# sarath-srinivas/PyGPR

Measured on AMD Instinct MI355X. Metric: NLML+grad evals/sec at N=16384 D=8 RBF, higher is better.
Workload: dtype f64; 1 GPU; BASELINE config 3: one exact-GP NLML+gradient evaluation per GPU per step, N=16384 D=8, Compose([Squared_exponential, White_noise]), hp sigma=1 l=1 sigma_n=0.1, jitter 1e-7; N>1: grBCM shared-hp co-training (each rank's expert = 1024 global + 15360 own points), one all-reduce of [1+nhp] per step; experts_per_gpu=1

## Files before the change

### pygpr_amd/_ops.py

```python
import atexit
import ctypes as C
import os

import torch

from . import _lib
from ._lib import PAD, PG_F32, PG_F64, CovSpec

JITTER = 1e-7


def pad_to(n, q=PAD):
    return ((int(n) + q - 1) // q) * q


def _code(dtype):
    if dtype == torch.float64:
        return PG_F64
    if dtype == torch.float32:
        return PG_F32
    raise TypeError("pygpr_amd computes in float64 or float32, got %s" % dtype)


def _p(t):
# ... 354 lines not shown
            "pg_trmm_lower_kt_batched")

    def syrk_nt_sub_batched(self, vt_all, c_all, lower_only=True):
        self._chk(vt_all, c_all)
        assert vt_all.dim() == 3 and c_all.dim() == 3 and vt_all.shape[0] == c_all.shape[0]
        _lib.check(self.lib.pg_syrk_nt_sub_batched(self.h, _code(c_all.dtype), c_all.shape[1], vt_all.shape[2], _p(vt_all),
                                                   vt_all.stride(1), vt_all.stride(0), _p(c_all), c_all.stride(1), c_all.stride(0),
                                                   c_all.shape[0], int(lower_only), self._st()), "pg_syrk_nt_sub_batched")

    def grbcm_local_terms(self, mean_c, var_c, var_g, is_first, accumulate, out, beta=None, prec=None):
        self._chk(mean_c, var_c, var_g, out, beta, prec)
        assert out.dtype == torch.float64 and out.shape[0] == 3
        _lib.check(self.lib.pg_grbcm_local_terms(self.h, _code(mean_c.dtype), mean_c.numel(), _p(mean_c), _p(var_c),
                                                 _p(var_g), int(is_first), int(accumulate), _p(out), out.stride(0),
                                                 _p(beta), _p(prec), self._st()), "pg_grbcm_local_terms")

    def grbcm_local_terms_batched(self, mean_all, var_all, var_g, first, accumulate, out, beta=None, prec=None):
        self._chk(var_g, out)
        assert out.dtype == torch.float64 and out.shape[0] == 3 and mean_all.stride(-1) == 1 and var_all.stride(-1) == 1
        m = var_g.numel()
        nexp = mean_all.shape[0]
        if beta is not None:
            assert beta.stride(-1) == 1 and prec.stride(-1) == 1 and (nexp == 1 or beta.stride(0) == prec.stride(0))
        _lib.check(self.lib.pg_grbcm_local_terms_batched(
            self.h, _code(mean_all.dtype), m, _p(mean_all), mean_all.stride(0), _p(var_all), var_all.stride(0), _p(var_g), nexp, int(first),
            int(accumulate), _p(out), out.stride(0), _p(beta), _p(prec), beta.stride(0) if beta is not None else 0, self._st()),
            "pg_grbcm_local_terms_batched")

    def grbcm_finish(self, sums, mean_g, var_g, mean, var, beta0=None, prec0=None):
        self._chk(sums, mean_g, var_g, mean, var, beta0, prec0)
        _lib.check(self.lib.pg_grbcm_finish(self.h, _code(mean_g.dtype), mean_g.numel(), _p(sums), sums.stride(0),
                                            _p(mean_g), _p(var_g), _p(mean), _p(var), _p(beta0), _p(prec0),
                                            self._st()), "pg_grbcm_finish")

    def grbcm_weighted_prec(self, prec, beta, acc, m, accumulate):
        self._chk(prec, beta, acc)
        _lib.check(self.lib.pg_grbcm_weighted_prec(self.h, _code(acc.dtype), m, acc.shape[0], _p(prec), prec.stride(0), _p(beta),
                                                   _p(acc), acc.stride(0), int(accumulate), self._st()), "pg_grbcm_weighted_prec")

    def symmetrize(self, a, n):
        self._chk(a)
        _lib.check(self.lib.pg_symmetrize(self.h, _code(a.dtype), n, _p(a), a.stride(0), self._st()), "pg_symmetrize")

    def grbcm_finish_full(self, sums, mean_g, var_g, cov, mean):
        self._chk(sums, mean_g, var_g, cov, mean)
        _lib.check(self.lib.pg_grbcm_finish_full(self.h, _code(mean_g.dtype), mean_g.numel(), _p(sums), sums.stride(0), _p(mean_g),
                                                 _p(var_g), _p(cov), cov.stride(0), _p(mean), self._st()), "pg_grbcm_finish_full")

    def spd_inverse_lower(self, a_pad):
        n = a_pad.shape[0]
        invd = self.potrf_workspace(n, a_pad.dtype)
        info = torch.zeros(1, dtype=torch.int32, device=self.device)
        self.potrf(a_pad, invd, info)
        minv = self.empty(n, n, dtype=a_pad.dtype)
        self.trtri(a_pad, invd, minv)
        out = self.empty(n, n, dtype=a_pad.dtype)
        self.lauum(minv, out)
        return out, info

    def spd_inverse_lower_batched(self, a_all):
        nexp, n = a_all.shape[0], a_all.shape[1]
        invd = self.empty(nexp, self.potrf_worksize(n, a_all.dtype), dtype=a_all.dtype)
        info = torch.zeros(nexp, dtype=torch.int32, device=self.device)
        minv = self.empty(nexp, n, n, dtype=a_all.dtype)
        self.potrf_trtri_batched(a_all, invd, info, minv)
        self.lauum_batched(minv, a_all)
        return a_all, info

    def sqdist_argmin(self, x, centres, dist=None, idx=None):
        self._chk(x, centres, dist, idx)
        _lib.check(self.lib.pg_sqdist_argmin(self.h, _code(x.dtype), _p(x), x.stride(0), x.shape[0], _p(centres),
                                             centres.stride(0), centres.shape[0], x.shape[1], _p(dist),
                                             dist.stride(0) if dist is not None else 0, _p(idx), self._st()), "pg_sqdist_argmin")

    def gemm_raw(self, variant, m, n, k, alpha, a, b, beta, c, tri=0, klo=0, khi=0):
        self._chk(a, b, c)
        _lib.check(self.lib.pg_gemm_raw(self.h, _code(c.dtype), variant, m, n, k, float(alpha), _p(a), a.stride(0),
                                        _p(b), b.stride(0), float(beta), _p(c), c.stride(0), tri, klo, khi,
                                        self._st()), "pg_gemm_raw")

    def set_lookahead(self, on):
        _lib.check(self.lib.pg_set_lookahead(self.h, int(on)), "pg_set_lookahead")

    def set_outer_panel(self, columns):
        _lib.check(self.lib.pg_set_outer_panel(self.h, int(columns)), "pg_set_outer_panel")

    def set_recursive_split(self, min_n):
        _lib.check(self.lib.pg_set_recursive_split(self.h, int(min_n)), "pg_set_recursive_split")

    def set_coupled_chain(self, on):
        _lib.check(self.lib.pg_set_coupled_chain(self.h, int(on)), "pg_set_coupled_chain")

    def set_spin_budget(self, microseconds):
        _lib.check(self.lib.pg_set_spin_budget(self.h, int(microseconds)), "pg_set_spin_budget")

    def chain_timeouts(self):
        return int(self.lib.pg_chain_timeouts(self.h))

    def set_rearm_after(self, calls):
        _lib.check(self.lib.pg_set_rearm_after(self.h, int(calls)), "pg_set_rearm_after")

    def chain_rearms(self):
        return int(self.lib.pg_chain_rearms(self.h))

    def wait_budget_us(self, n):
        return int(self.lib.pg_wait_budget_us(self.h, int(n)))

    def spin_probe(self, n):
        scratch = torch.zeros(4, dtype=torch.int64, device=self.device)
        _lib.check(self.lib.pg_spin_probe(self.h, int(n), _p(scratch), self._st()), "pg_spin_probe")
        torch.cuda.synchronize()
        v = scratch.tolist()
        return v[2] * 1e-5, bool(v[3])

    def recover_from_timeout(self):
        torch.cuda.synchronize()
        self.chain_timeouts()
        if self.coupled_chain():
            _lib.check(self.lib.pg_set_coupled_chain(self.h, -1), "pg_set_coupled_chain")
        self.fallbacks = getattr(self, "fallbacks", 0) + 1

    def build_factor_checked(self, spec, hp, x, a, invd, info, minv=None, jitter=JITTER):
        passes = _passes(spec)
        assert len(passes) == 1
        self._chk(hp, x, a, invd, info, minv)
        n, d = x.shape
        out = C.c_int(0)
        _lib.check(self.lib.pg_build_potrf_trtri_checked(
            self.h, _code(a.dtype), C.byref(passes[0]), _p(hp), _p(x), x.stride(0), n, d, float(jitter), _p(a), a.stride(0),
            a.shape[0], _p(invd), _p(info), _p(minv), minv.stride(0) if minv is not None else 0, self._st(), C.byref(out)),
            "pg_build_potrf_trtri_checked")
        return out.value

    def coupled_chain(self):
        return int(self.lib.pg_coupled_chain(self.h))

    def last_coupled_panels(self):
        return int(self.lib.pg_last_coupled_panels(self.h))

    def leaf_raw(self, a, inv, info):
        self._chk(a, inv, info)
        _lib.check(self.lib.pg_leaf_raw(self.h, _code(a.dtype), _p(a), a.stride(0), _p(inv), inv.stride(0) if inv is not None else 0,
                                        _p(info), self._st()), "pg_leaf_raw")

    def profile(self, on):
        _lib.check(self.lib.pg_profile(self.h, int(on)), "pg_profile")

    def profile_read(self):
        f, ms, n = C.c_double(), C.c_double(), C.c_long()
        _lib.check(self.lib.pg_profile_read(self.h, C.byref(f), C.byref(ms), C.byref(n)), "pg_profile_read")
        return f.value, ms.value, n.value


_OPS = None


def get_ops():
    global _OPS
    if _OPS is None:
        _OPS = HipOps()
    return _OPS


def _passes(spec):
    return spec if isinstance(spec, (list, tuple)) else [spec]

# ... 20 lines not shown
```

### pygpr_amd/csrc/capi.hip

```cpp
#include "gemm.h"
#include "kbuild.h"
#include "leaf.h"
#include "chainstep.h"
#include "linalg.h"
#include <cstdarg>
#include <cstdint>
#include <cstdio>
#include <cstdlib>
#include <cstring>
#include <mutex>
#include <vector>

static thread_local char g_err[512] = "";

static std::mutex g_live_mu;
static std::vector<pg_ctx*> g_live;
static bool g_atexit_registered = false;

static void release_ctx(pg_ctx* h) {
    (void)hipStreamDestroy(h->aux);
    if (h->rows) (void)hipStreamDestroy(h->rows);
    if (h->upd) (void)hipStreamDestroy(h->upd);
    for (int i = 0; i < 8; ++i) (void)hipEventDestroy(h->ev[i]);
    for (int i = 0; i < h->npool; ++i) (void)hipEventDestroy(h->pool[i]);
// ... 123 lines not shown
static int probe_concurrent_queues(pg_ctx* c) {
    if (!c->probe_words && hipHostMalloc(reinterpret_cast<void**>(&c->probe_words), 64, hipHostMallocMapped) != hipSuccess) {
        (void)hipGetLastError();
        c->probe_words = nullptr;
        return 0;
    }
    int* words = c->probe_words;
    words[0] = 0;
    words[1] = 0;
    int* dwords = nullptr;
    int ok = 0;
    if (hipHostGetDevicePointer(reinterpret_cast<void**>(&dwords), words, 0) == hipSuccess) {
        hipLaunchKernelGGL(pg_probe_wait_kernel, dim3(1), dim3(1), 0, c->aux, dwords, dwords + 1);
        hipLaunchKernelGGL(pg_probe_set_kernel, dim3(1), dim3(1), 0, c->rows, dwords);
        if (hipStreamSynchronize(c->aux) == hipSuccess && hipStreamSynchronize(c->rows) == hipSuccess) ok = words[1] == 1;
    }
    (void)hipGetLastError();
    return ok;
}

static void maybe_rearm(pg_ctx* h) {
    if (h && h->coupled && h->rearms > 0 && h->rearm_cur > h->rearm_after && ++h->calls_since_rearm > h->rearm_cur) {
        h->rearm_cur = h->rearm_after;
        h->calls_since_rearm = 0;
    }
    if (!h || !h->tmo_off || h->coupled || h->rearm_after <= 0) return;
    if (h->rearm_cur < h->rearm_after) h->rearm_cur = h->rearm_after;
    if (++h->calls_since_tmo <= h->rearm_cur) return;
    h->calls_since_tmo = 0;
    if (h->rows && h->spin_ticks >= 0 && probe_concurrent_queues(h)) {
        h->coupled = 1;
        h->tmo_off = 0;
        h->rearms += 1;
        h->calls_since_rearm = 0;
    }
}

template <typename T>
static int build_potrf_t(pg_handle h, hipStream_t st, const pg_covspec* spec, const double* hp, const void* X, long ldx, int n, int d,
                         double jitter, void* A, long lda, int n_pad, void* inv_diag, int* info, void* Minv, long ldm) {
    BuildReq<T> br;
    br.spec = spec; br.hp = hp; br.X = (const T*)X; br.ldx = ldx; br.n_real = n; br.d = d; br.jitter = jitter;
    return pg_potrf_t<T>(h, st, n_pad, (T*)A, lda, (T*)inv_diag, info, (T*)Minv, ldm, &br);
}

template <typename T>
static int potrf_batched_t(pg_handle h, hipStream_t st, const pg_covspec* spec, const double* hp, long hp_stride, const void* X, long ldx,
                           long x_stride, int n, int d, double jitter, void* A, long lda, long a_stride, int n_pad, void* inv_diag,
                           long inv_stride, int* info, void* Minv, long ldm, long m_stride, int nexp) {
    ExpBatch eb;
    eb.nexp = nexp; eb.eA = a_stride; eb.eInv = inv_stride; eb.eM = m_stride; eb.eX = x_stride; eb.ehp = hp_stride;
    BuildReq<T> br;
    br.spec = spec; br.hp = hp; br.X = (const T*)X; br.ldx = ldx; br.n_real = n; br.d = d; br.jitter = jitter;
    return pg_potrf_t<T>(h, st, n_pad, (T*)A, lda, (T*)inv_diag, info, (T*)Minv, ldm, X ? &br : nullptr, &eb);
}

extern "C" {

int pg_version(void) { return 100; }
const char* pg_last_error(void) { return g_err; }

int pg_create(pg_handle* h) {
    NEED(h, "null handle pointer");
    int count = 0;
    if (hipGetDeviceCount(&count) != hipSuccess || count == 0) {
        pg_set_error("pg_create: no HIP device visible");
        return -101;
    }
    pg_ctx* c = new pg_ctx();
    memset(c, 0, sizeof(*c));
    int prio_lo = 0, prio_hi = 0;
    PG_CHECK(hipDeviceGetStreamPriorityRange(&prio_lo, &prio_hi));
    PG_CHECK(hipStreamCreateWithPriority(&c->aux, hipStreamNonBlocking, prio_hi));
    c->rows = nullptr;
    c->last_coupled = 0;
    c->lookahead = 1;
    {
        const char* e = getenv("PG_NBO");
        c->nbo = e ? atoi(e) : 0;
        if (c->nbo < 128 || c->nbo % 128 || c->nbo > 2048) c->nbo = 0;
        const char* r = getenv("PG_REC_MIN");
        c->rec_min = r ? atoi(r) : 16384;
        if (c->rec_min < 0 || (c->rec_min > 0 && (c->rec_min < 512 || c->rec_min % 512))) c->rec_min = 16384;
    }
    {
        hipDeviceProp_t prop;
        int dev = 0;
        PG_CHECK(hipGetDevice(&dev));
        PG_CHECK(hipGetDeviceProperties(&prop, dev));
        const int ncu = prop.multiProcessorCount;
        const int words = (ncu + 31) / 32;
        uint32_t mask[64];
        for (int i = 0; i < 64; ++i) mask[i] = 0;
        const char* env = getenv("PG_RESERVED_CUS");
        int reserved = env ? atoi(env) : PG_RESERVED_CUS;
        if (reserved < 1 || reserved > ncu / 2) reserved = PG_RESERVED_CUS;
        c->ncu = ncu; c->upd_cus = ncu - reserved;
        for (int cu = 0; cu < ncu - reserved; ++cu) mask[cu / 32] |= (1u << (cu % 32));
        if (ncu <= reserved * 2 || words > 64 ||
            hipExtStreamCreateWithCUMask(&c->upd, (uint32_t)words, mask) != hipSuccess) {
            c->upd = nullptr;
            c->lookahead = 0;
            (void)hipGetLastError();
        }
    }
    {
        const char* envr = getenv("PG_ROWS_STREAM");
        c->rows = nullptr;
        if (!(envr && !atoi(envr)) && c->upd &&
            hipStreamCreateWithPriority(&c->rows, hipStreamNonBlocking, prio_hi) != hipSuccess) {
            c->rows = nullptr;
            (void)hipGetLastError();
        }
    }
    c->coupled = (c->rows && probe_concurrent_queues(c)) ? 1 : 0;
    {
        c->tmo_host = nullptr;
        c->tmo_dev = nullptr;
        if (hipHostMalloc(reinterpret_cast<void**>(&c->tmo_host), 64, hipHostMallocMapped) == hipSuccess) {
            c->tmo_host[0] = 0;
            if (hipHostGetDevicePointer(reinterpret_cast<void**>(&c->tmo_dev), c->tmo_host, 0) != hipSuccess) c->tmo_dev = nullptr;
        }
        (void)hipGetLastError();
        const char* e = getenv("PG_CS_SPIN_US");
        const long long us = e ? atoll(e) : 0;
        c->spin_ticks = us < 0 ? -1 : us * 100;
        c->timeouts = 0;
        const char* ra = getenv("PG_CS_REARM");
        c->rearm_after = ra ? std::max(0, atoi(ra)) : 8;
        c->rearm_cur = c->rearm_after;
    }
    for (int i = 0; i < 8; ++i) PG_CHECK(hipEventCreate(&c->ev[i]));
    {
        std::lock_guard<std::mutex> lk(g_live_mu);
        g_live.push_back(c);
        if (!g_atexit_registered) {
            atexit(destroy_live_handles);
            g_atexit_registered = true;
        }
    }
    *h = c;
    return 0;
}

int pg_destroy(pg_handle h) {
    if (!h) return 0;
    {
        std::lock_guard<std::mutex> lk(g_live_mu);
        auto it = std::find(g_live.begin(), g_live.end(), h);
        if (it == g_live.end()) return 0;
        g_live.erase(it);
    }
    release_ctx(h);
    return 0;
}

static int check_spec(const pg_covspec* s, const char* fn, bool allow_sqdist = false) {
    if (!s || s->ncomp < 0 || s->ncomp > PG_MAX_COMP || s->nnoise < 0 || s->nnoise > PG_MAX_COMP) {
        pg_set_error("%s: bad covariance spec", fn);
        return -1;
    }
    for (int c = 0; c < s->ncomp; ++c)
        if (s->kind[c] != PG_KIND_RBF && s->kind[c] != PG_KIND_MATERN52 && s->kind[c] != PG_KIND_MATERN32 && s->kind[c] != PG_KIND_MATERN12 &&
            !(allow_sqdist && s->kind[c] == PG_KIND_SQDIST)) {
            pg_set_error("%s: unknown kernel kind %d", fn, s->kind[c]);
            return -1;
// ... 456 lines not shown
}

int pg_grbcm_local_terms(pg_handle h, int dtype, int m, const void* mean_c, const void* var_c, const void* var_g,
                         int is_first, int accumulate, double* out, long ldo, double* beta_out, double* prec_out,
                         void* stream) {
    JOIN(h, stream);
    NEED(h && mean_c && var_c && var_g && out, "null pointer");
    NEED(ldo >= m, "ldo < m");
    DISPATCH(dtype,
             pg_grbcm_terms_t<double>(ST(stream), m, (const double*)mean_c, (const double*)var_c, (const double*)var_g,
                                      is_first, accumulate, out, ldo, beta_out, prec_out),
             pg_grbcm_terms_t<float>(ST(stream), m, (const float*)mean_c, (const float*)var_c, (const float*)var_g,
                                     is_first, accumulate, out, ldo, beta_out, prec_out));
}

int pg_grbcm_local_terms_batched(pg_handle h, int dtype, int m, const void* mean_l, long mean_stride, const void* var_l, long var_stride,
                                 const void* var_g, int nexp, int first, int accumulate, double* out, long ldo, double* beta_out,
                                 double* prec_out, long ldb, void* stream) {
    JOIN(h, stream);
    NEED(h && mean_l && var_l && var_g && out, "null pointer");
    NEED(ldo >= m && nexp >= 1 && (nexp == 1 || (!beta_out && !prec_out) || ldb >= m), "bad size");
    DISPATCH(dtype,
             pg_grbcm_terms_batched_t<double>(ST(stream), m, (const double*)mean_l, mean_stride, (const double*)var_l, var_stride,
                                              (const double*)var_g, nexp, first, accumulate, out, ldo, beta_out, prec_out, ldb),
             pg_grbcm_terms_batched_t<float>(ST(stream), m, (const float*)mean_l, mean_stride, (const float*)var_l, var_stride,
                                             (const float*)var_g, nexp, first, accumulate, out, ldo, beta_out, prec_out, ldb));
}

int pg_grbcm_finish(pg_handle h, int dtype, int m, const double* sums, long lds, const void* mean_g, const void* var_g,
                    void* mean, void* var, double* beta0, double* prec0, void* stream) {
    JOIN(h, stream);
    NEED(h && sums && mean_g && var_g && mean && var, "null pointer");
    DISPATCH(dtype,
             pg_grbcm_finish_t<double>(ST(stream), m, sums, lds, (const double*)mean_g, (const double*)var_g, (double*)mean,
                                       (double*)var, beta0, prec0),
             pg_grbcm_finish_t<float>(ST(stream), m, sums, lds, (const float*)mean_g, (const float*)var_g, (float*)mean,
                                      (float*)var, beta0, prec0));
}

int pg_grbcm_weighted_prec(pg_handle h, int dtype, int m, int m_pad, const void* P, long ldp, const double* beta, void* acc,
                           long lda, int accumulate, void* stream) {
    JOIN(h, stream);
    NEED(h && P && beta && acc, "null pointer");
    NEED(m_pad >= m && ldp >= m && lda >= m_pad, "inconsistent sizes");
    DISPATCH(dtype, pg_weighted_prec_t<double>(ST(stream), m, m_pad, (const double*)P, ldp, beta, (double*)acc, lda, accumulate),
             pg_weighted_prec_t<float>(ST(stream), m, m_pad, (const float*)P, ldp, beta, (float*)acc, lda, accumulate));
}

int pg_symmetrize(pg_handle h, int dtype, int n, void* A, long lda, void* stream) {
    JOIN(h, stream);
    NEED(h && A, "null pointer");
    DISPATCH(dtype, pg_symmetrize_t<double>(ST(stream), n, (double*)A, lda), pg_symmetrize_t<float>(ST(stream), n, (float*)A, lda));
}

int pg_grbcm_finish_full(pg_handle h, int dtype, int m, const double* sums, long lds, const void* mean_g, const void* var_g,
                         const void* cov, long ldc, void* mean, void* stream) {
    JOIN(h, stream);
    NEED(h && sums && mean_g && var_g && cov && mean, "null pointer");
    DISPATCH(dtype,
             pg_grbcm_finish_full_t<double>(ST(stream), m, sums, lds, (const double*)mean_g, (const double*)var_g,
                                            (const double*)cov, ldc, (double*)mean),
             pg_grbcm_finish_full_t<float>(ST(stream), m, sums, lds, (const float*)mean_g, (const float*)var_g, (const float*)cov,
                                           ldc, (float*)mean));
}

int pg_sqdist_argmin(pg_handle h, int dtype, const void* X, long ldx, int n, const void* C, long ldc, int m, int d, void* D,
                     long ldd, int* idx, void* stream) {
    JOIN(h, stream);
    NEED(h && X && C && (D || idx), "null pointer");
    DISPATCH(dtype,
             pg_centres<double>(ST(stream), (const double*)X, ldx, n, (const double*)C, ldc, m, d, (double*)D, ldd, idx),
             pg_centres<float>(ST(stream), (const float*)X, ldx, n, (const float*)C, ldc, m, d, (float*)D, ldd, idx));
}

int pg_tril(pg_handle h, int dtype, int n, void* A, long lda, void* stream) {
    JOIN(h, stream);
    NEED(h && A, "null pointer");
    DISPATCH(dtype, pg_tril_t<double>(ST(stream), n, (double*)A, lda), pg_tril_t<float>(ST(stream), n, (float*)A, lda));
}

int pg_set_lookahead(pg_handle h, int on) {
    NEED(h, "null handle");
    h->lookahead = (on && h->upd) ? 1 : 0;
    return 0;
}

int pg_set_outer_panel(pg_handle h, int columns) {
    NEED(h, "null handle");
    NEED(columns == 0 || (columns >= 128 && columns % 128 == 0 && columns <= 2048), "outer panel must be 0 (automatic) or a multiple of 128 up to 2048");
    h->nbo = columns;
    return 0;
}

int pg_set_recursive_split(pg_handle h, int min_n) {
    NEED(h, "null handle");
    NEED(min_n == 0 || (min_n >= 512 && min_n % 512 == 0), "min_n must be 0 (never) or a multiple of 512");
    h->rec_min = min_n;
    return 0;
}

int pg_profile(pg_handle h, int on) {
    NEED(h, "null handle");
    if (on) { h->prof_flops = 0; h->prof_ms = 0; h->prof_launches = 0; }
    h->prof_on = on;
    return 0;
}
int pg_set_coupled_chain(pg_handle h, int on) {
    NEED(h, "null handle");
    if (on < 0) {
        if (h->coupled || h->tmo_off == 0) { h->tmo_off = h->rows ? 1 : 0; h->calls_since_tmo = 0; }
        h->coupled = 0;
        return 0;
    }
    h->tmo_off = 0;
    h->rearm_cur = h->rearm_after;
    h->rearms_seen = h->rearms;
    h->calls_since_rearm = 0;
    if (!on) {
        if (h->rows) {
            PG_CHECK(hipStreamSynchronize(h->rows));
            PG_CHECK(hipStreamDestroy(h->rows));
            h->rows = nullptr;
        }
        h->coupled = 0;
        return 0;
    }
    if (!h->rows && h->upd) {
        int prio_lo = 0, prio_hi = 0;
        PG_CHECK(hipDeviceGetStreamPriorityRange(&prio_lo, &prio_hi));
        if (hipStreamCreateWithPriority(&h->rows, hipStreamNonBlocking, prio_hi) != hipSuccess) {
            h->rows = nullptr;
            (void)hipGetLastError();
        }
    }
    h->coupled = (h->rows && probe_concurrent_queues(h)) ? 1 : 0;
    return 0;
}
int pg_coupled_chain(pg_handle h) { return h ? h->coupled : -1; }
int pg_last_coupled_panels(pg_handle h) {
    if (!h) return -1;
    return h->last_coupled;
}
int pg_profile_read(pg_handle h, double* flops, double* ms, long* launches) {
    NEED(h, "null handle");
    if (flops) *flops = h->prof_flops;
    if (ms) *ms = h->prof_ms;
    if (launches) *launches = h->prof_launches;
    return 0;
}

int pg_set_spin_budget(pg_handle h, long microseconds) {
    NEED(h, "null handle");
    h->spin_ticks = microseconds < 0 ? -1 : (long long)microseconds * 100;
    return 0;
}
int pg_set_rearm_after(pg_handle h, int calls) {
    NEED(h, "null handle");
    NEED(calls >= 0, "calls must be >= 0 (0: never re-arm automatically)");
    h->rearm_after = calls;
    h->rearm_cur = calls;
    h->rearms_seen = h->rearms;
    h->calls_since_rearm = 0;
    return 0;
}
int pg_chain_rearms(pg_handle h) { return h ? h->rearms : -1; }
long pg_wait_budget_us(pg_handle h, int n) {
// ... 68 lines not shown
```

### pygpr_amd/csrc/common.h

```cpp
#pragma once
#include <hip/hip_runtime.h>
#include <stdint.h>
#include <algorithm>
#include "pygpr_hip.h"

#define PG_TILE 128
#define PG_RESERVED_CUS 32
#define PG_PAD 256


typedef double pg_d4 __attribute__((ext_vector_type(4)));
typedef float pg_f4 __attribute__((ext_vector_type(4)));

struct pg_ctx {
    hipStream_t aux;
    hipStream_t rows;
    hipStream_t upd;
    hipEvent_t ev[8];
    hipEvent_t* pool;
    int npool;
    int lookahead;
    int nbo;
    int rec_min;
    int coupled;
    int last_coupled;
    int side_pending;
    hipStream_t side_owner;
    int* tmo_host;
    int* tmo_dev;
    long long spin_ticks;
    int timeouts;
    int tmo_off;
    int calls_since_tmo;
    int rearm_after;
    int rearms;
    int rearms_seen;
    int rearm_cur;
    int calls_since_rearm;
    int* probe_words;
    int chain_epoch;
    int counted_epoch;
    int no_atomic_c;
    int ncu, upd_cus;
    int prof_on;
    double prof_flops;
    double prof_ms;
    long prof_launches;
};

void pg_set_error(const char* fmt, ...);

#define PG_CHECK(expr)                                                              \
    do {                                                                            \
        hipError_t _e = (expr);                                                     \
        if (_e != hipSuccess) {                                                     \
            pg_set_error("%s:%d %s -> %s", __FILE__, __LINE__, #expr,               \
                         hipGetErrorString(_e));                                    \
            return -100;                                                            \
        }                                                                           \
    } while (0)

template <typename T> struct Mfma;
template <> struct Mfma<double> {
    typedef pg_d4 acc_t;
    static __device__ __forceinline__ acc_t run(double a, double b, acc_t c) {
        return __builtin_amdgcn_mfma_f64_16x16x4f64(a, b, c, 0, 0, 0);
    }
    static __device__ __forceinline__ int row(int lane, int r) { return (lane >> 4) + 4 * r; }
};
template <> struct Mfma<float> {
    typedef pg_f4 acc_t;
    static __device__ __forceinline__ acc_t run(float a, float b, acc_t c) {
        return __builtin_amdgcn_mfma_f32_16x16x4f32(a, b, c, 0, 0, 0);
    }
    static __device__ __forceinline__ int row(int lane, int r) { return (lane >> 4) * 4 + r; }
};

template <typename T> __device__ __forceinline__ T wave_sum(T v) {
#pragma unroll
    for (int o = 32; o > 0; o >>= 1) v += __shfl_xor(v, o, 64);
    return v;
}
```

### pygpr_amd/csrc/linalg.hip

```cpp
#include "gemm.h"
#include "leaf.h"
#include "chainstep.h"
#include "kbuild.h"
#include "linalg.h"
#include <cmath>
#include <cstdlib>
#include <vector>

#define NB 128
static int pg_nbo(const pg_ctx* ctx, int n) {
    if (ctx->nbo) return ctx->nbo;
    return n <= 10240 ? 512 : (n <= 18432 ? 1024 : 2048);
}

template <typename T>
__global__ __launch_bounds__(256) void copy_blocks_kernel(const T* __restrict__ src, T* __restrict__ dst, long ldd, long esrc, long edst) {
    src += blockIdx.z * esrc;
    dst += blockIdx.z * edst;
    const int b = blockIdx.x;
    const T* s = src + (long)b * NB * NB;
    T* d = dst + (long)b * NB * ldd + (long)b * NB;
    for (int idx = blockIdx.y * 256 + threadIdx.x; idx < NB * NB; idx += gridDim.y * 256)
        d[(long)(idx >> 7) * ldd + (idx & 127)] = s[idx];
}
// ... 291 lines not shown
    const int tc = blockIdx.x, tr = blockIdx.y;
    if (tc < tr) return;
    for (int idx = threadIdx.x; idx < 64 * 64; idx += 256) {
        const int i = tr * 64 + (idx >> 6), j = tc * 64 + (idx & 63);
        if (i < n && j < n && j > i) A[(long)i * lda + j] = A[(long)j * lda + i];
    }
}

template <typename T>
__global__ __launch_bounds__(256) void grbcm_finish_full_kernel(const double* __restrict__ sums, long lds, const T* __restrict__ mean_g,
                                                                const T* __restrict__ var_g, const T* __restrict__ cov, long ldc,
                                                                int m, T* __restrict__ mean) {
    const int j = blockIdx.x * 256 + threadIdx.x;
    if (j >= m) return;
    const double pg = 1.0 / (double)var_g[j];
    const double b0 = 1.0 - sums[j];
    mean[j] = (T)((double)cov[(long)j * ldc + j] * (sums[2 * lds + j] + b0 * pg * (double)mean_g[j]));
}

#define LAUNCH_CHECK() PG_CHECK(hipGetLastError())

template <typename T> static GemmP<T> gp0() {
    GemmP<T> p;
    p.A = p.B = nullptr; p.C = nullptr;
    p.lda = p.ldb = p.ldc = 0;
    p.M = p.N = p.K = 0;
    p.alpha = (T)1; p.beta = (T)0;
    p.tri = p.klo = p.khi = 0; p.krev = 0;
    p.sA = p.sB = p.sC = 0; p.batch = 1;
    p.nexp = 1; p.eA = p.eB = p.eC = 0; p.einfo = 0;
    p.part = nullptr; p.ldp = 0; p.info = nullptr; p.noxcd = 0;
    return p;
}

static long pg_flag_elems(int n) { return 128L * (n / NB) + 2048; }
long pg_potrf_worksize_impl(int n) { return (long)n * NB + pg_flag_elems(n); }

template <typename T>
int pg_trtri_t(pg_ctx* ctx, hipStream_t st, int n, const T* L, long ldl, const T* invD, T* M, long ldm, int hmax, const ExpBatch* eb) {
    if (n <= 0 || n % NB) { pg_set_error("pg_trtri: n=%d is not a positive multiple of %d", n, NB); return -2; }
    const int nexp = eb ? eb->nexp : 1;
    const long eL = eb ? eb->eA : 0, eI = eb ? eb->eInv : 0, eMm = eb ? eb->eM : 0;
    hipLaunchKernelGGL(copy_blocks_kernel<T>, dim3(n / NB, 8, nexp), dim3(256), 0, st, invD, M, ldm, eI, eMm);
    LAUNCH_CHECK();
    int rc;
    long h = NB, rem = 0;
    for (;;) {
        const long nfull = (n - rem) / h;
        if (nfull + (rem ? 1 : 0) <= 1) break;
        if (hmax && h >= hmax) break;
        const long npair = nfull / 2;
        for (int pass = 0; pass < 2; ++pass) {
            long r0, h2, batch;
            if (pass == 0) { if (!npair) continue; r0 = 0; h2 = h; batch = npair; }
            else { if (!((nfull & 1) && rem)) continue; r0 = (nfull - 1) * h; h2 = rem; batch = 1; }
            const long stride = 2 * h * (ldm + 1);
            GemmP<T> p = gp0<T>();
            p.M = (int)h; p.N = (int)h2; p.K = (int)h;
            p.A = M + r0 * ldm + r0; p.lda = ldm;
            p.B = L + (r0 + h) * ldl + r0; p.ldb = ldl;
            p.C = M + r0 * ldm + r0 + h; p.ldc = ldm;
            p.klo = 1; p.batch = (int)batch;
            p.sA = stride; p.sC = stride; p.sB = 2 * h * (ldl + 1);
            p.nexp = nexp; p.eA = eMm; p.eB = eL; p.eC = eMm;
            const bool small = batch * (h / 128) * (h2 / 128) * nexp <= 1024 && h2 % 64 == 0;
            if ((rc = pg_gemm<T>(ctx, st, small ? GEMM_TT_64 : GEMM_TT_128, p))) return rc;
            p = gp0<T>();
            p.M = (int)h2; p.N = (int)h; p.K = (int)h2;
            p.A = M + (r0 + h) * ldm + r0 + h; p.lda = ldm;
            p.B = M + r0 * ldm + r0 + h; p.ldb = ldm;
            p.C = M + (r0 + h) * ldm + r0; p.ldc = ldm;
            p.alpha = (T)-1; p.khi = 1; p.batch = (int)batch;
            p.sA = p.sB = p.sC = stride;
            p.nexp = nexp; p.eA = p.eB = p.eC = eMm;
            if ((rc = pg_gemm<T>(ctx, st, small ? GEMM_NT_64 : GEMM_NT_128, p))) return rc;
        }
        if (nfull & 1) rem = rem ? h + rem : h;
        h *= 2;
    }
    return 0;
}

template <typename T>
static int trtri_top(pg_ctx* ctx, hipStream_t st, int h1, int h2, const T* L, long ldl, T* M, long ldm) {
    int rc;
    GemmP<T> p = gp0<T>();
    p.M = h1; p.N = h2; p.K = h1; p.A = M; p.lda = ldm; p.B = L + (long)h1 * ldl; p.ldb = ldl; p.C = M + h1; p.ldc = ldm; p.klo = 1;
    if ((rc = pg_gemm<T>(ctx, st, GEMM_TT_128, p))) return rc;
    p = gp0<T>();
    p.M = h2; p.N = h1; p.K = h2; p.A = M + (long)h1 * ldm + h1; p.lda = ldm; p.B = M + h1; p.ldb = ldm;
    p.C = M + (long)h1 * ldm; p.ldc = ldm; p.alpha = (T)-1; p.khi = 1;
    return pg_gemm<T>(ctx, st, GEMM_NT_128, p);
}

long long pg_wait_ticks(const pg_ctx* ctx, int n) {
    if (ctx->spin_ticks != 0) return ctx->spin_ticks;
    const double est_us = 62.0 * (n / NB) + (double)n * n * n / 3.0 / 35.0e6;
    return (long long)(std::max(50000.0, 20.0 * est_us) * 100.0);
}

static int pool_event(pg_ctx* ctx, int idx, hipEvent_t* ev) {
    if (idx >= ctx->npool) {
        const int want = idx + 16;
        hipEvent_t* p = (hipEvent_t*)realloc(ctx->pool, sizeof(hipEvent_t) * want);
        if (!p) { pg_set_error("out of memory for events"); return -3; }
        ctx->pool = p;
        for (int i = ctx->npool; i < want; ++i) PG_CHECK(hipEventCreateWithFlags(&ctx->pool[i], hipEventDisableTiming));
        ctx->npool = want;
    }
    *ev = ctx->pool[idx];
    return 0;
}

template <typename T>
int pg_potrf_t(pg_ctx* ctx, hipStream_t st, int n, T* A, long lda, T* invD, int* info, T* Minv, long ldm, const BuildReq<T>* build,
               const ExpBatch* eb, int col_off, int keep_info);

static int pg_rec_split(const pg_ctx* ctx, int n) {
    if (ctx->rec_min <= 0 || n < ctx->rec_min || n < 2 * PG_PAD) return 0;
    return ((n / 2 + PG_PAD - 1) / PG_PAD) * PG_PAD;
}

template <typename T>
static int potrf_trtri_rec(pg_ctx* ctx, hipStream_t st, int n, T* A, long lda, T* invD, int* info, T* Minv, long ldm,
                           const BuildReq<T>* build, int col_off) {
    const int h1 = pg_rec_split(ctx, n), h2 = n - h1;
    int rc;
    T* A21 = A + (long)h1 * lda;
    T* A22 = A21 + h1;
    T* M21 = Minv + (long)h1 * ldm;
    BuildReq<T> b1;
    if (build) { b1 = *build; b1.n_real = std::min(build->n_real, h1); }
    const bool side = build && ctx->lookahead && !ctx->prof_on && ctx->upd;
    if (side) PG_CHECK(hipEventRecord(ctx->ev[0], st));
    if ((rc = pg_potrf_t<T>(ctx, st, h1, A, lda, invD, info, Minv, ldm, build ? &b1 : nullptr, nullptr, col_off, 1))) return rc;
    if (build) {
        const int nr2 = std::max(0, build->n_real - h1);
        const T* X2 = build->X + (long)h1 * build->ldx;
        hipStream_t bs = side ? ctx->upd : st;
        if (side) PG_CHECK(hipStreamWaitEvent(bs, ctx->ev[0], 0));
        if ((rc = pg_kbuild<T>(bs, *build->spec, build->hp, X2, build->ldx, nr2, build->X, build->ldx, std::min(build->n_real, h1), build->d,
                               0, 0, 0, 0.0, M21, ldm, h2, h1)))
            return rc;
        if ((rc = pg_kbuild<T>(bs, *build->spec, build->hp, X2, build->ldx, nr2, X2, build->ldx, nr2, build->d, 1, 1, 0, build->jitter, A22,
                               lda, h2, h2)))
            return rc;
        if (side) {
            PG_CHECK(hipEventRecord(ctx->ev[1], bs));
            PG_CHECK(hipStreamWaitEvent(st, ctx->ev[1], 0));
        }
    } else {
        const long vecs = (long)h2 * h1 / (16 / sizeof(T));
        hipLaunchKernelGGL(copy_rows_kernel<T>, dim3((unsigned)std::min<long>((vecs + 255) / 256, 8192)), dim3(256), 0, st, A21, lda, M21, ldm,
                           h2, h1);
        LAUNCH_CHECK();
    }
    {
        GemmP<T> p = gp0<T>(); p.info = info;
        p.M = h2; p.N = h1; p.K = h1; p.A = M21; p.lda = ldm; p.B = Minv; p.ldb = ldm; p.C = A21; p.ldc = lda; p.khi = 2;
        if ((rc = pg_gemm<T>(ctx, st, GEMM_NT_128, p))) return rc;
    }
    {
        GemmP<T> p = gp0<T>(); p.info = info;
        p.M = p.N = h2; p.K = h1; p.A = A21; p.lda = lda; p.B = A21; p.ldb = lda; p.C = A22; p.ldc = lda;
        p.alpha = (T)-1; p.beta = (T)1; p.tri = 1;
        if ((rc = pg_gemm<T>(ctx, st, GEMM_NT_128, p))) return rc;
    }
    if ((rc = pg_potrf_t<T>(ctx, st, h2, A22, lda, invD + (long)(h1 / NB) * NB * NB, info, Minv + (long)h1 * ldm + h1, ldm, nullptr, nullptr,
                            col_off + h1, 1)))
        return rc;
    return trtri_top<T>(ctx, st, h1, h2, A, lda, Minv, ldm);
}

#define COUPLED_ROWS 8192
#define COUPLED_PANEL 384
#define U_SMALL_ROWS 8192
#define SB_SMALL_TILES 2048
template <typename T>
int pg_potrf_t(pg_ctx* ctx, hipStream_t st, int n, T* A, long lda, T* invD, int* info, T* Minv, long ldm, const BuildReq<T>* build,
               const ExpBatch* eb, int col_off, int keep_info) {
    if (n <= 0 || n % PG_PAD) { pg_set_error("pg_potrf: n=%d is not a positive multiple of %d", n, PG_PAD); return -2; }
    const int nexp = eb ? eb->nexp : 1;
    const long eA = eb ? eb->eA : 0, eI = eb ? eb->eInv : 0;
    if (nexp < 1) { pg_set_error("pg_potrf: empty batch"); return -2; }
    auto batched = [&](GemmP<T>& p, long sa, long sb, long sc) { p.nexp = nexp; p.eA = sa; p.eB = sb; p.eC = sc; p.einfo = nexp > 1 ? 1 : 0; };
    if (!keep_info) PG_CHECK(hipMemsetAsync(info, 0, sizeof(int) * nexp, st));
    if (Minv && nexp == 1 && pg_rec_split(ctx, n) > 0) return potrf_trtri_rec<T>(ctx, st, n, A, lda, invD, info, Minv, ldm, build, col_off);
    const int NBO = pg_nbo(ctx, n);
    hipStream_t rows_stream = ctx->rows;
    static const int cs_batched = getenv("PG_CS_BATCHED") ? atoi(getenv("PG_CS_BATCHED")) : 1;
    const bool batch_cp = cs_batched && nexp <= 24 && (cs_batched == 2 || (n >= 2048 && (long)nexp * n <= 24576));
    const bool want_cp = ctx->lookahead && !ctx->prof_on && ctx->coupled && rows_stream && (nexp == 1 || batch_cp);
    std::vector<int> pb;
    for (int c = 0; c < n;) {
        pb.push_back(c);
        c += (want_cp && n - c <= COUPLED_ROWS) ? std::min(NBO, COUPLED_PANEL) : NBO;
    }
    pb.push_back(n);
    const int npan = (int)pb.size() - 1;
    const bool la = ctx->lookahead && !ctx->prof_on && npan >= 3;
    hipStream_t ps = la ? ctx->aux : st;
    hipStream_t us = la ? ctx->upd : st;
    hipEvent_t ev;
    int rc;
    const bool build_split = build && la && npan >= 2;
    if (build) {
        const int c1 = build_split ? pb[1] : n;
        if ((rc = pg_kbuild<T>(st, *build->spec, build->hp, build->X, build->ldx, build->n_real, build->X, build->ldx, build->n_real,
                               build->d, 1, 1, 0, build->jitter, A, lda, n, n, 0, c1, nexp, eb ? eb->eX : 0, eb ? eb->ehp : 0, eA)))
            return rc;
    }
    if (la) {
        if ((rc = pool_event(ctx, 0, &ev))) return rc;
        PG_CHECK(hipEventRecord(ev, st));
        PG_CHECK(hipStreamWaitEvent(ps, ev, 0));
        PG_CHECK(hipStreamWaitEvent(us, ev, 0));
    }
    if (build_split) {
        if ((rc = pg_kbuild<T>(us, *build->spec, build->hp, build->X, build->ldx, build->n_real, build->X, build->ldx, build->n_real,
                               build->d, 1, 1, 0, build->jitter, A, lda, n, n, pb[1], n, nexp, eb ? eb->eX : 0, eb ? eb->ehp : 0, eA)))
            return rc;
        if ((rc = pool_event(ctx, 7 + 2 * npan, &ev))) return rc;
        PG_CHECK(hipEventRecord(ev, us));
    }
    T* flagw = invD + (long)n * NB;
    const bool coupled = la && want_cp;
    int o_s = npan;
    if (coupled)
        for (int o = 0; o < npan; ++o)
            if (n - pb[o] <= COUPLED_ROWS) { o_s = o; break; }
    ctx->last_coupled = npan - o_s;
    const int nblk = n / NB;
    int* f_diag = reinterpret_cast<int*>(flagw);
    int* f_done = f_diag + nblk;
    int* f_brow = f_done + nblk;
    int* f_early = f_brow + nblk;
    int* f_browe = f_early + nblk;
    int* f_tmo = f_browe + nblk;
    if (o_s < npan) ctx->chain_epoch = ctx->chain_epoch % 1000000 + 1;
    const CsWait cw = {f_tmo, ctx->tmo_dev, pg_wait_ticks(ctx, n), ctx->chain_epoch};
    const CsBatch cbat = {nexp, eA, eI, (long)(eI * (long)sizeof(T) / (long)sizeof(int))};
    if (o_s < npan) {
        PG_CHECK(hipMemset2DAsync(f_diag, (size_t)(nexp > 1 ? eI : pg_potrf_worksize_impl(n)) * sizeof(T), 0, (size_t)((5 * nblk + 1 + 3) / 4) * 16, (size_t)nexp, ps));
    }
    std::vector<char> nf_split(npan + 1, 0);
    for (int o = 0; o < npan; ++o) {
        const int o0 = pb[o], oend = pb[o + 1];
        const bool cp = o >= o_s;
        if (cp) {
            hipStream_t rs = rows_stream;
            if (o == o_s) {
                if ((rc = pg_flagset(ps, f_diag + o0 / NB, PG_CS_NCRIT, nexp, cbat.eF))) return rc;
                if ((rc = pool_event(ctx, 4 + 2 * npan, &ev))) return rc;
                PG_CHECK(hipEventRecord(ev, ps));
// ... 512 lines not shown
```

Baseline: 13.82 evals/s.

## Overlap part of top-block triangular inverse GEMM with trailing Cholesky on side stream

In the recursive potrf+trtri path, the first GEMM of the top-half inverse update (M·L21ᵀ) is split by columns. A share of those columns is issued on the CU-masked update stream right after the trailing A22 update, so it runs concurrently with the recursive factorisation of A22, and the main stream picks up the rest. The share comes from a heuristic that depends on h1 and dtype, and an environment variable can override it. The cost is extra events and cross-stream waits, plus contention for CUs between the two streams.

Result: no change. 13.73 evals/s (-0.6%).

```diff
diff --git a/pygpr_amd/_ops.py b/pygpr_amd/_ops.py
--- a/pygpr_amd/_ops.py
+++ b/pygpr_amd/_ops.py
@@ -460,6 +460,9 @@
     def set_lookahead(self, on):
         _lib.check(self.lib.pg_set_lookahead(self.h, int(on)), "pg_set_lookahead")
 
+    def set_split_overlap(self, on):
+        _lib.check(self.lib.pg_set_lookahead(self.h, 1 if on else 2), "pg_set_lookahead")
+
     def set_outer_panel(self, columns):
         _lib.check(self.lib.pg_set_outer_panel(self.h, int(columns)), "pg_set_outer_panel")
 
diff --git a/pygpr_amd/csrc/capi.hip b/pygpr_amd/csrc/capi.hip
--- a/pygpr_amd/csrc/capi.hip
+++ b/pygpr_amd/csrc/capi.hip
@@ -229,6 +229,10 @@
         const char* r = getenv("PG_REC_MIN");
         c->rec_min = r ? atoi(r) : 16384;
         if (c->rec_min < 0 || (c->rec_min > 0 && (c->rec_min < 512 || c->rec_min % 512))) c->rec_min = 16384;
+        const char* ss = getenv("PG_SPLIT_SIDE");
+        c->split_overlap = 1;
+        c->split_side = ss ? atoi(ss) : 0;
+        if (c->split_side < 0 || c->split_side > 8) c->split_side = 0;
     }
     {
         hipDeviceProp_t prop;
@@ -851,6 +855,7 @@
 int pg_set_lookahead(pg_handle h, int on) {
     NEED(h, "null handle");
     h->lookahead = (on && h->upd) ? 1 : 0;
+    h->split_overlap = on == 2 ? 0 : 1;
     return 0;
 }
 
diff --git a/pygpr_amd/csrc/common.h b/pygpr_amd/csrc/common.h
--- a/pygpr_amd/csrc/common.h
+++ b/pygpr_amd/csrc/common.h
@@ -22,6 +22,8 @@
     int lookahead;
     int nbo;
     int rec_min;
+    int split_overlap;
+    int split_side;
     int coupled;
     int last_coupled;
     int side_pending;
diff --git a/pygpr_amd/csrc/linalg.hip b/pygpr_amd/csrc/linalg.hip
--- a/pygpr_amd/csrc/linalg.hip
+++ b/pygpr_amd/csrc/linalg.hip
@@ -397,12 +397,16 @@
 }
 
 template <typename T>
-static int trtri_top(pg_ctx* ctx, hipStream_t st, int h1, int h2, const T* L, long ldl, T* M, long ldm) {
-    int rc;
+static int trtri_top_s(pg_ctx* ctx, hipStream_t st, int h1, int c0, int c1, const T* L, long ldl, T* M, long ldm, int* info) {
+    if (c1 <= c0) return 0;
+    GemmP<T> p = gp0<T>(); p.info = info;
+    p.M = h1; p.N = c1 - c0; p.K = h1; p.A = M; p.lda = ldm; p.B = L + (long)(h1 + c0) * ldl; p.ldb = ldl; p.C = M + h1 + c0; p.ldc = ldm;
+    p.klo = 1;
+    return pg_gemm<T>(ctx, st, GEMM_TT_128, p);
+}
+template <typename T>
+static int trtri_top_m21(pg_ctx* ctx, hipStream_t st, int h1, int h2, T* M, long ldm) {
     GemmP<T> p = gp0<T>();
-    p.M = h1; p.N = h2; p.K = h1; p.A = M; p.lda = ldm; p.B = L + (long)h1 * ldl; p.ldb = ldl; p.C = M + h1; p.ldc = ldm; p.klo = 1;
-    if ((rc = pg_gemm<T>(ctx, st, GEMM_TT_128, p))) return rc;
-    p = gp0<T>();
     p.M = h2; p.N = h1; p.K = h2; p.A = M + (long)h1 * ldm + h1; p.lda = ldm; p.B = M + h1; p.ldb = ldm;
     p.C = M + (long)h1 * ldm; p.ldc = ldm; p.alpha = (T)-1; p.khi = 1;
     return pg_gemm<T>(ctx, st, GEMM_NT_128, p);
@@ -430,6 +434,13 @@
 template <typename T>
 int pg_potrf_t(pg_ctx* ctx, hipStream_t st, int n, T* A, long lda, T* invD, int* info, T* Minv, long ldm, const BuildReq<T>* build,
                const ExpBatch* eb, int col_off, int keep_info);
+
+static int pg_split_side_cols(const pg_ctx* ctx, int h1, int h2, size_t elem) {
+    double share = (elem == 8 ? 0.42 : 0.83) * (8192.0 / h1) * (8192.0 / h1);
+    if (ctx->split_side > 0) share = ctx->split_side / 8.0;
+    const int tc = h2 / NB;
+    return NB * std::min(tc, std::max(1, (int)(share * tc + 0.5)));
+}
 
 static int pg_rec_split(const pg_ctx* ctx, int n) {
     if (ctx->rec_min <= 0 || n < ctx->rec_min || n < 2 * PG_PAD) return 0;
@@ -481,10 +492,26 @@
         p.alpha = (T)-1; p.beta = (T)1; p.tri = 1;
         if ((rc = pg_gemm<T>(ctx, st, GEMM_NT_128, p))) return rc;
     }
+    const bool ovl = ctx->split_overlap && ctx->lookahead && !ctx->prof_on && ctx->upd;
+    const int evb = 10 + 4 * (h1 / NB);
+    hipEvent_t ev_a22 = nullptr, ev_s = nullptr;
+    if (ovl) {
+        if ((rc = pool_event(ctx, evb, &ev_a22))) return rc;
+        if ((rc = pool_event(ctx, evb + 1, &ev_s))) return rc;
+        PG_CHECK(hipEventRecord(ev_a22, st));
+    }
     if ((rc = pg_potrf_t<T>(ctx, st, h2, A22, lda, invD + (long)(h1 / NB) * NB * NB, info, Minv + (long)h1 * ldm + h1, ldm, nullptr, nullptr,
                             col_off + h1, 1)))
         return rc;
-    return trtri_top<T>(ctx, st, h1, h2, A, lda, Minv, ldm);
+    const int ns = ovl ? pg_split_side_cols(ctx, h1, h2, sizeof(T)) : 0;
+    if (ns > 0) {
+        PG_CHECK(hipStreamWaitEvent(ctx->upd, ev_a22, 0));
+        if ((rc = trtri_top_s<T>(ctx, ctx->upd, h1, 0, ns, A, lda, Minv, ldm, info))) return rc;
+        PG_CHECK(hipEventRecord(ev_s, ctx->upd));
+    }
+    if ((rc = trtri_top_s<T>(ctx, st, h1, ns, h2, A, lda, Minv, ldm, info))) return rc;
+    if (ns > 0) PG_CHECK(hipStreamWaitEvent(st, ev_s, 0));
+    return trtri_top_m21<T>(ctx, st, h1, h2, Minv, ldm);
 }
 
 #define COUPLED_ROWS 8192
```
